# robotic-vision-lab/Dual-Interactive-Implicit-Neural-Network

Hardware: AMD Instinct MI355X
Metric: decoded Mpixels/sec (DIINN implicit decoder, x4 on 256^2 LR) (higher is better)
Workload: dtype f32

## Files before the change

dual-interactive-implicit-neural-network_amd/_native.py:

```python
from __future__ import annotations

import ctypes as C
import os
import threading

PKG_DIR = os.path.dirname(os.path.abspath(__file__))
LIB_PATH = os.environ.get("DIINN_HIP_LIB") or os.path.join(PKG_DIR, "libdiinn_hip.so")

DIINN_OK = 0
ERR_INVALID_ARG, ERR_UNSUPPORTED, ERR_HIP, ERR_TOO_LARGE = 1, 2, 3, 4
SIN_ACCURATE = 0
SIN_HW = 1
SIN_HW_REDUCED = 2
SIN_DEFAULT = SIN_HW_REDUCED
ABI_VERSION = 10
PACKED_MAGIC = 0x44493038
PACKED_MAGIC_WPU = 0x44495750
P_ALGO_DIRECT, P_ALGO_WINOGRAD, P_ALGO_DIRECT_BF16, P_ALGO_DIRECT_BF16X3 = 0, 1, 2, 3
RDN_ALGO_AUTO, RDN_ALGO_DIRECT, RDN_ALGO_WINO, RDN_ALGO_WINO4, RDN_ALGO_X3 = 0, 1, 2, 3, 4
COMPUTE_F32 = 0
COMPUTE_BF16 = 1
COMPUTE_F32_QONLY = 2
COMPUTE_BF16_FULL = 3
COMPUTE_BF16X3 = 4
# ... 56 lines not shown
    "diinn_metasr_decode": (C.c_int, [C.c_void_p, C.c_void_p, C.c_void_p, C.c_void_p, C.c_void_p,
                                      C.c_int, C.c_int, C.c_int, C.c_int, C.c_int]),
    "diinn_metasr_make_axis_tables": (C.c_int, [C.c_int, C.c_int, _i32, _f, _f]),
    "diinn_conv_ksplit": (C.c_int, [C.c_void_p, C.c_void_p, C.c_longlong, C.c_int, C.c_int, C.c_void_p, C.c_void_p,
                                   C.c_void_p, C.c_longlong, C.c_void_p, C.c_longlong, C.c_void_p, C.c_longlong,
                                   C.c_int, C.c_int, C.c_int, C.c_int]),
    "diinn_rdn_packed_floats": (C.c_size_t, []),
    "diinn_rdn_planes_floats": (C.c_size_t, [C.c_int, C.c_int, C.c_int, C.c_int]),
    "diinn_rdn_forward_ex": (C.c_int, [C.c_void_p, C.c_int, C.c_void_p, C.c_void_p, C.c_void_p, C.c_void_p, C.c_void_p, C.c_void_p,
                                       C.c_void_p, C.c_void_p, C.c_void_p, C.c_int, C.c_int, C.c_int]),
    "diinn_conv_wino4_ws_status": (C.c_int, [C.c_void_p, C.c_void_p, C.c_int, _ip]),
    "diinn_sfe1_forward": (C.c_int, [C.c_void_p, C.c_void_p, C.c_int, C.c_void_p, C.c_void_p, C.c_void_p,
                                    C.c_int, C.c_int, C.c_int]),
    "diinn_conv_wino": (C.c_int, [C.c_void_p, C.c_void_p, C.c_longlong, C.c_int, C.c_void_p, C.c_void_p,
                                 C.c_void_p, C.c_longlong, C.c_void_p, C.c_longlong, C.c_int, C.c_int, C.c_int, C.c_int]),
    "diinn_conv3x3_x3": (C.c_int, [C.c_void_p, C.c_void_p, C.c_longlong, C.c_int, C.c_void_p, C.c_void_p,
                                   C.c_void_p, C.c_longlong, C.c_void_p, C.c_longlong, C.c_int, C.c_int, C.c_int, C.c_int]),
    "diinn_rdn_x3_packed_floats": (C.c_size_t, []),
    "diinn_conv_t16": (C.c_int, [C.c_void_p, C.c_void_p, C.c_longlong, C.c_int, C.c_void_p, C.c_void_p,
                                C.c_void_p, C.c_longlong, C.c_void_p, C.c_longlong, C.c_int, C.c_int, C.c_int, C.c_int]),
    "diinn_conv_t16_applies": (C.c_int, [C.c_int, C.c_int, C.c_int]),
    "diinn_conv_t16_plan": (C.c_int, [C.c_int, C.c_int, C.c_int, C.POINTER(C.c_int)]),
    "diinn_conv1x1_t16": (C.c_int, [C.c_void_p, C.c_void_p, C.c_longlong, C.c_int, C.c_void_p, C.c_void_p,
                                   C.c_void_p, C.c_longlong, C.c_void_p, C.c_longlong, C.c_void_p, C.c_longlong,
                                   C.c_int, C.c_int, C.c_int, C.c_int]),
    "diinn_rdn_wino_packed_floats": (C.c_size_t, []),
    "diinn_conv_wino4": (C.c_int, [C.c_void_p, C.c_void_p, C.c_longlong, C.c_int, C.c_void_p, C.c_void_p,
                                  C.c_void_p, C.c_longlong, C.c_void_p, C.c_longlong, C.c_int, C.c_int, C.c_int, C.c_int]),
    "diinn_conv_wino4_ws": (C.c_int, [C.c_void_p, C.c_void_p, C.c_longlong, C.c_int, C.c_void_p, C.c_void_p,
                                     C.c_void_p, C.c_longlong, C.c_void_p, C.c_longlong, C.c_int, C.c_int, C.c_int, C.c_int,
                                     C.c_void_p, C.c_size_t]),
    "diinn_conv_wino4_workspace_floats": (C.c_size_t, []),
    "diinn_conv_wino4_plan": (C.c_int, [C.c_int, C.c_int, C.c_int, C.c_int, C.c_int, C.POINTER(C.c_int)]),
    "diinn_rdn_wino4_packed_floats": (C.c_size_t, []),
    "diinn_rdn_wino4_applies": (C.c_int, [C.c_int, C.c_int, C.c_int]),
    "diinn_liif_decode": (C.c_int, [C.c_void_p, C.c_void_p, C.c_void_p, C.c_void_p, C.c_void_p,
                                    C.c_int, C.c_int, C.c_int, C.c_int, C.c_int]),
    "diinn_liif_make_axis_tables": (C.c_int, [C.c_int, C.c_int, C.c_int, _i32, _f, _f]),
    "diinn_backward_data": (C.c_int, [C.c_void_p, C.c_void_p, C.c_void_p, C.c_void_p, C.c_void_p, C.c_void_p,
                                      C.c_longlong]),
    "diinn_plane_gemm_nt": (C.c_int, [C.c_void_p, C.c_void_p, C.c_int, C.c_int, C.c_void_p, C.c_int, C.c_int,
                                      C.c_void_p, C.c_int, C.c_int, C.c_longlong, C.c_int, C.c_int]),
    "diinn_plane_rowdot": (C.c_int, [C.c_void_p, C.c_void_p, C.c_int, C.c_void_p, C.c_void_p, C.c_int,
                                     C.c_longlong, C.c_int]),
    "diinn_backward_cell_sum": (C.c_int, [C.c_void_p, C.c_void_p, C.c_void_p, C.c_void_p, C.c_void_p,
                                          C.c_int, C.c_int, C.c_int, C.c_int, C.c_int]),
    "diinn_sum_parts": (C.c_int, [C.c_void_p, C.c_void_p, C.c_void_p, C.c_int, C.c_int, C.c_longlong]),
    "diinn_backward_cell_sum_ex": (C.c_int, [C.c_void_p, C.c_void_p, C.c_void_p, C.c_void_p, C.c_void_p, C.c_void_p,
                                             C.c_int, C.c_int, C.c_int, C.c_int, C.c_int]),
    "diinn_unfold_tiled": (C.c_int, [C.c_void_p, C.c_void_p, C.c_void_p, C.c_int, C.c_int, C.c_int, C.c_int]),
    "diinn_training_plane_floats": (C.c_longlong, [C.c_longlong, C.c_int]),
    "diinn_decode_train_fwd": (C.c_int, [C.c_void_p, C.c_void_p, C.c_void_p, C.c_void_p, C.c_void_p,
                                         C.c_int, C.c_int, C.c_int, C.c_int, C.c_int, C.c_int]),
}

_lib = None
_lock = threading.Lock()


class DiinnNativeError(RuntimeError):
    pass


def load() -> C.CDLL:
    global _lib
    if _lib is not None:
# ... 45 lines not shown
```

dual-interactive-implicit-neural-network_amd/csrc/diinn_device.h:

```cpp
#pragma once
#include <hip/hip_runtime.h>
#include <stdint.h>

#include "../../include/diinn_hip.h"
#include "diinn_layout.h"
#include "diinn_knobs.h"

using namespace diinn;

typedef float f32x4 __attribute__((ext_vector_type(4)));
typedef float f32x16 __attribute__((ext_vector_type(16)));
typedef float f32x2 __attribute__((ext_vector_type(2)));
typedef unsigned u32x2 __attribute__((ext_vector_type(2)));
template <int N> struct IC { static constexpr int value = N; };

#define MFMA32(a, b, c) __builtin_amdgcn_mfma_f32_32x32x2f32((a), (b), (c), 0, 0, 0)

template <int MODE>
__device__ __forceinline__ float dsin(float x);

template <>
__device__ __forceinline__ float dsin<DIINN_SIN_ACCURATE>(float x) {
    const float k = __builtin_rintf(x * 0.31830988618379067154f);
    float r = __builtin_fmaf(k, -3.14159274101257324219f, x);
// ... 117 lines not shown
}
struct BlockXYZ { int x, y, z; };
__device__ __forceinline__ BlockXYZ xcd_run_block() {
    const unsigned gx = gridDim.x, gy = gridDim.y;
    const unsigned total = gx * gy * gridDim.z, full = total & ~7u;
    const unsigned lin = blockIdx.x + gx * (blockIdx.y + gy * blockIdx.z);
    const unsigned t = lin < full ? (lin & 7u) * (full >> 3) + (lin >> 3) : lin;
    const unsigned z = t / (gx * gy), r = t - z * gx * gy, y = r / gx;
    return BlockXYZ{__builtin_amdgcn_readfirstlane((int)(r - y * gx)), __builtin_amdgcn_readfirstlane((int)y), __builtin_amdgcn_readfirstlane((int)z)};
}

__device__ __forceinline__ void st_b128(f32x4 v, __amdgpu_buffer_rsrc_t rsrc, unsigned voff, unsigned soff) {
    __builtin_amdgcn_raw_buffer_store_b128(__builtin_bit_cast(u32x4, v), rsrc, (int)voff, (int)soff, 0);
    asm volatile("s_nop 1" ::"v"(v[0]), "v"(v[1]), "v"(v[2]), "v"(v[3]));
}
__device__ __forceinline__ float ld_act(__amdgpu_buffer_rsrc_t rsrc, unsigned voff, unsigned soff) {
    return __builtin_bit_cast(float, __builtin_amdgcn_raw_buffer_load_b32(rsrc, (int)voff, (int)soff, 0));
}
__device__ __forceinline__ __amdgpu_buffer_rsrc_t tile_rsrc(const float* group, long long tile, int rows) {
    return __builtin_amdgcn_make_buffer_rsrc((void*)(group + (size_t)tile * rows * PLANE_TILE), 0,
                                             rows * (int)PLANE_ROW_BYTES, 0x00020000);
}

typedef __bf16 bf16x8 __attribute__((ext_vector_type(8)));
#define MFMA_BF16(a, b, c) __builtin_amdgcn_mfma_f32_32x32x16_bf16((a), (b), (c), 0, 0, 0)

__attribute__((visibility("hidden"))) extern thread_local int g_last_hip_error;
#ifdef DIINN_STAMPS
extern unsigned long long* g_stamps;
#endif

__attribute__((visibility("hidden"))) int device_cus();
__attribute__((visibility("hidden"))) double w4_rounds(long long total, bool have_ws);

static inline int hip_status(hipError_t e) {
    if (e == hipSuccess) return DIINN_OK;
    g_last_hip_error = (int)e;
    return DIINN_ERR_HIP;
}

static inline bool compute_ok(int compute) {
    return compute == DIINN_COMPUTE_F32 || compute == DIINN_COMPUTE_BF16 || compute == DIINN_COMPUTE_F32_QONLY ||
           compute == DIINN_COMPUTE_BF16_FULL || compute == DIINN_COMPUTE_BF16X3;
}

__device__ __forceinline__ int div_m(int x, int d, unsigned m) { return m ? (int)(((unsigned long long)(unsigned)x * m) >> 32) : x / d; }
static inline unsigned magic_m(long long d, long long x_max) { return (d > 1 && d < 65536 && x_max < 65536) ? (unsigned)((1ull << 32) / (unsigned long long)d + 1) : 0u; }
static inline int check_dims(int B, int H, int W) {
    if (B <= 0 || H <= 0 || W <= 0) return DIINN_ERR_INVALID_ARG;
    if ((double)B * H * W * PCH >= 9.0e18 || B > 65535 || H > 65535) return DIINN_ERR_TOO_LARGE;
    return DIINN_OK;
}

static inline int check_window(int row0, int rows, int full, int need0, int need1) {
    if (row0 < 0 || rows <= 0 || row0 > full - rows) return DIINN_ERR_INVALID_ARG;
    if (need0 < row0 || need1 > row0 + rows) return DIINN_ERR_INVALID_ARG;
    return DIINN_OK;
}

static inline int check_npix(long long npix) {
    if (npix <= 0) return DIINN_ERR_INVALID_ARG;
    if (npix > DIINN_TRAIN_MAX_PIXELS) return DIINN_ERR_TOO_LARGE;
    return DIINN_OK;
}

struct RowWin { int row0, rows; };
// ... 26 lines not shown
```

dual-interactive-implicit-neural-network_amd/csrc/diinn_encoder.hip:

```cpp
#include "diinn_device.h"

constexpr int CS_WAVES = 8;
constexpr int CS_TW = 8, CS_TH = 4;
constexpr int CS_HALO = (CS_TH + 2) * (CS_TW + 2);
constexpr int CS_STAGE_FLOATS = 2048;

struct TagFalse { static constexpr bool value = false; };
struct TagTrue { static constexpr bool value = true; };

struct ConvKsplitParams {
    const float* in;
    const float* w;
    const float* bias;
    const float* res;
    float* out0;
    float* out1;
    long long in_bs, out0_bs, out1_bs, res_bs;
    int Cin, B, H, W, relu;
    unsigned m_per_image, m_tiles_x;
#ifdef DIINN_STAMPS
    unsigned long long* stamps;
#endif
};

// ... 575 lines not shown

int diinn_rdn_forward_ex(void* stream, int algo, const float* sfe1_dev, const float* packed_dev, const float* packed_wino_dev,
                         const float* packed_wino4_dev, const float* packed_x3_dev, const float* biases_dev,
                         float* planes, float* w4ws, float* out_dev, int B, int H, int W) {
    switch (algo) {
        case DIINN_RDN_ALGO_AUTO: packed_x3_dev = nullptr; break;
        case DIINN_RDN_ALGO_DIRECT: packed_wino_dev = packed_wino4_dev = packed_x3_dev = nullptr; break;
        case DIINN_RDN_ALGO_WINO:
            if (!packed_wino_dev) return DIINN_ERR_INVALID_ARG;
            packed_wino4_dev = packed_x3_dev = nullptr;
            break;
        case DIINN_RDN_ALGO_WINO4:
            if (!packed_wino4_dev) return DIINN_ERR_INVALID_ARG;
            packed_x3_dev = nullptr;
            break;
        case DIINN_RDN_ALGO_X3:
            if (!packed_wino_dev || !packed_x3_dev) return DIINN_ERR_INVALID_ARG;
            packed_wino4_dev = nullptr;
            break;
        default: return DIINN_ERR_INVALID_ARG;
    }
    if ((((size_t)planes) & 15) || (((size_t)w4ws) & 15)) return DIINN_ERR_INVALID_ARG;
    if (!sfe1_dev || !packed_dev || !biases_dev || !planes || !out_dev) return DIINN_ERR_INVALID_ARG;
    int st = check_dims(B, H, W);
    if (st) return st;
    const long long hw = (long long)H * W;
    const long long wino_min = knob(diinn_knobs().enc_wino_min);
    const bool wino = (packed_wino_dev || packed_wino4_dev) && (long long)B * hw >= wino_min;
    const bool wino4 = packed_wino4_dev && wino && diinn_rdn_wino4_applies(B, H, W);
    if (wino && !wino4 && !packed_wino_dev) return DIINN_ERR_INVALID_ARG;
    const size_t w4ws_floats = w4ws ? diinn_conv_wino4_workspace_floats() : 0;
    if (wino4 && w4ws) {
        st = hip_status(hipMemsetAsync(w4ws, 0, DIINN_WINO4_COUNTER_BYTES, (hipStream_t)stream));
        if (st) return st;
    }
    float* buf[2] = {planes, planes + (size_t)B * 576 * hw};
    float* gff_in = planes + (size_t)2 * B * 576 * hw;
    float* tmp = gff_in + (size_t)B * 1024 * hw;
    const bool x3 = packed_x3_dev && (long long)B * hw >= knob(diinn_knobs().enc_x3_min);
    const bool t16 = !wino && !x3 && diinn_conv_t16_applies(B, H, W) != 0 &&
                     ((((size_t)sfe1_dev) | ((size_t)planes) | ((size_t)packed_dev)) & 15) == 0;
    RdnWeights wt{packed_dev, packed_wino_dev, packed_wino4_dev, packed_x3_dev, biases_dev};
    auto conv = [&](const float* in, long long in_bs, int cin, int taps, const float* res, long long res_bs,
                    float* o0, long long o0_bs, float* o1, long long o1_bs, int relu) {
        const RdnWeights::Slices l = wt.next(cin, taps);
        return (x3 && taps == 9 && !o1)
            ? diinn_conv3x3_x3(stream, in, in_bs, cin, l.wx, l.bias, res, res_bs, o0, o0_bs, relu, B, H, W)
            : (wino4 && taps == 9 && !o1)
            ? diinn_conv_wino4_ws(stream, in, in_bs, cin, l.wu4, l.bias, res, res_bs, o0, o0_bs, relu, B, H, W, w4ws, w4ws_floats)
            : (wino && taps == 9 && !o1)
            ? diinn_conv_wino(stream, in, in_bs, cin, l.wu, l.bias, res, res_bs, o0, o0_bs, relu, B, H, W)
            : (t16 && taps == 9 && !o1)
            ? diinn_conv_t16(stream, in, in_bs, cin, l.w, l.bias, res, res_bs, o0, o0_bs, relu, B, H, W)
            : (t16 && taps == 1 && cin <= 640)
            ? diinn_conv1x1_t16(stream, in, in_bs, cin, l.w, l.bias, res, res_bs, o0, o0_bs, o1, o1_bs, relu, B, H, W)
            : diinn_conv_ksplit(stream, in, in_bs, cin, taps, l.w, l.bias, res, res_bs, o0, o0_bs, o1, o1_bs, relu, B, H, W);
    };
    float* xs = tmp + (size_t)B * 64 * hw;
    const long long xs_bs16 = 144 * hw;
    if (x3) {
        const RdnWeights::Slices l = wt.next(64, 9);
        st = diinn_conv3x3_x3_split(stream, sfe1_dev, 64 * hw, xs, xs_bs16, 0, 64, l.wx, l.bias, buf[0], 576 * hw, 0, B, H, W);
    } else {
        st = conv(sfe1_dev, 64 * hw, 64, 9, nullptr, 0, buf[0], 576 * hw, nullptr, 0, 0);
    }
    if (st) return st;
    for (int d = 0; d < 16; ++d) {
        float* cur = buf[d & 1];
        float* nxt = buf[(d + 1) & 1];
        if (x3) {
            for (int c = 0; c < 8; ++c) {
                const RdnWeights::Slices l = wt.next(64 * (c + 1), 9);
                st = diinn_conv3x3_x3_split(stream, nullptr, 0, xs, xs_bs16, 8 * (c + 1), 64 * (c + 1), l.wx, l.bias,
                                            nullptr, 0, 1, B, H, W);
                if (st) return st;
            }
            const RdnWeights::Slices l = wt.next(576, 1);
            st = diinn_conv1x1_x3_split(stream, xs, xs_bs16, 576, l.wx, l.bias, cur, 576 * hw, nxt, 576 * hw,
                                        gff_in + (size_t)64 * d * hw, 1024 * hw, B, H, W);
            if (st) return st;
            continue;
        }
        for (int c = 0; c < 8; ++c) {
            st = conv(cur, 576 * hw, 64 * (c + 1), 9, nullptr, 0, cur + (size_t)64 * (c + 1) * hw, 576 * hw, nullptr, 0, 1);
            if (st) return st;
        }
        st = conv(cur, 576 * hw, 576, 1, cur, 576 * hw, nxt, 576 * hw, gff_in + (size_t)64 * d * hw, 1024 * hw, 0);
        if (st) return st;
    }
    st = conv(gff_in, 1024 * hw, 1024, 1, nullptr, 0, tmp, 64 * hw, nullptr, 0, 0);
    if (st) return st;
    return conv(tmp, 64 * hw, 64, 9, sfe1_dev, 64 * hw, out_dev, 64 * hw, nullptr, 0, 0);
}

}
```

dual-interactive-implicit-neural-network_amd/csrc/diinn_winograd4.hip:

```cpp
#include "diinn_device.h"

constexpr int W4_TX = 32;
constexpr int W4_THREADS = 1024;
constexpr int W4_VBUF = 36 * 256;
constexpr int W4_RAW0 = 3 * W4_VBUF;
constexpr int W4_RAW_WAVE = 6 * 256 + 64;
constexpr int W4_LDS_FLOATS = W4_RAW0 + 2 * 4 * W4_RAW_WAVE;
static_assert(W4_LDS_FLOATS >= 36 * 1024 && W4_LDS_FLOATS * 4 <= 160 * 1024, "LDS budget");
constexpr int W4_PIECE_BYTES = 1024;
static_assert(3 * W4_VBUF <= W4_LDS_FLOATS, "ring inside the exchange buffer");

#pragma clang diagnostic ignored "-Winline-asm"
#define W4_SB() __builtin_amdgcn_sched_barrier(0)
typedef int i32x4 __attribute__((ext_vector_type(4)));
__device__ __forceinline__ i32x4 w4_rsrc(const void* ptr, unsigned bytes) {
    const unsigned long long a = (unsigned long long)ptr;
    return i32x4{(int)(unsigned)a, (int)((unsigned)(a >> 32) & 0xffffu), (int)bytes, 0x00020000};
}

struct ConvWino4Params {
    const float* in;
    const float* wu;
    const float* bias;
    const float* res;
// ... 43 lines not shown
static_assert(DIINN_WINO4_MAX_SPLIT_WGS <= W4_READY, "one ticket and one ready word per split item");

struct W4Split { int parts, item, slab, first_pair, pair, blk_item; };

__device__ __forceinline__ void w4_st_sc1(f32x4 v, __amdgpu_buffer_rsrc_t rsrc, unsigned voff) {
    __builtin_amdgcn_raw_buffer_store_b128(__builtin_bit_cast(u32x4, v), rsrc, (int)voff, 0, 16);
}
__device__ __forceinline__ f32x4 w4_ld_sc1(__amdgpu_buffer_rsrc_t rsrc, unsigned voff) {
    return __builtin_bit_cast(f32x4, __builtin_amdgcn_raw_buffer_load_b128(rsrc, (int)voff, 0, 16));
}

template <typename T>
__device__ __forceinline__ void w4_bt(const T d0, const T d1, const T d2, const T d3, const T d4, const T d5,
                                      T& r0, T& r1, T& r2, T& r3, T& r4, T& r5) {
    const T a = __builtin_elementwise_fma(T(-4.0f), d2, d4), b = __builtin_elementwise_fma(T(-4.0f), d1, d3);
    const T c = d4 - d2, e = d3 - d1;
    r0 = __builtin_elementwise_fma(T(4.0f), d0, __builtin_elementwise_fma(T(-5.0f), d2, d4));
    r1 = a + b;
    r2 = a - b;
    r3 = __builtin_elementwise_fma(T(2.0f), e, c);
    r4 = __builtin_elementwise_fma(T(-2.0f), e, c);
    r5 = __builtin_elementwise_fma(T(4.0f), d1, __builtin_elementwise_fma(T(-5.0f), d3, d5));
}
template <typename T>
__device__ __forceinline__ void w4_at(const T m0, const T m1, const T m2, const T m3, const T m4, const T m5,
                                      T& y0, T& y1, T& y2, T& y3) {
    const T s = m1 + m2, d = m1 - m2, u = m3 + m4, v = m3 - m4;
    y0 = (m0 + s) + u;
    y1 = __builtin_elementwise_fma(T(2.0f), v, d);
    y2 = __builtin_elementwise_fma(T(4.0f), u, s);
    y3 = __builtin_elementwise_fma(T(8.0f), v, d) + m5;
}

__device__ __forceinline__ void conv_wino4_body(const ConvWino4Params& p, float* __restrict__ lds, int b, int blk, int hh0,
                                                int c0, int m, const W4Split sk) {
    const int tiles_x = (p.W + 3) / 4, tiles_n = tiles_x * ((p.H + 3) / 4);
    auto tile_xy = [&](int tile, int& tx, int& ty) {
        ty = div_m(tile, tiles_x, p.m_tiles_x);
        tx = tile - ty * tiles_x;
        return tile < tiles_n;
    };
    const int lane = threadIdx.x & 63;
    const int wave = __builtin_amdgcn_readfirstlane(threadIdx.x >> 6);
    const size_t plane = (size_t)p.H * p.W;
    const unsigned plane_b = (unsigned)(plane * sizeof(float));
    const int n = p.Cin / 8;
    constexpr unsigned OUTSIDE = 0x80000000u;
    const bool ragged = (p.W & 3) != 0;

    const bool producer = (wave & 3) == 3;
    const int wt_ = wave >> 2, mw = (wave >> 2) * 3 + (wave & 3);
    if (threadIdx.x == 0) W4_STAMP(0, 76, 0);
    if (producer) {
        const int wt = wt_;
        __builtin_amdgcn_s_setprio(3);
        const int th = lane >> 5, tm = lane & 31;
        int ptx, pty;
        const bool pin = tile_xy(blk * W4_TX + tm, ptx, pty);
        (void)pin;
        const bool first = tm == 0, last = tm == W4_TX - 1;
        const bool row_start = ptx == 0, row_end = 4 * ptx + 4 >= p.W;
        const bool ok1 = 4 * ptx + 1 < p.W, ok2 = 4 * ptx + 2 < p.W, ok3 = 4 * ptx + 3 < p.W;
        float* __restrict__ raw = lds + W4_RAW0 + wt * W4_RAW_WAVE;
        const float* __restrict__ in_b = p.in + (size_t)b * p.in_bs;
        unsigned voff[6], voffe;
        {
            const int ek = lane % 6, ew = lane / 6;
            int etx, ety;
// ... 41 lines not shown
                w4_bt<f32x2>(d[0][j], d[1][j], d[2][j], d[3][j], d[4][j], d[5][j], t[0][j], t[1][j], t[2][j], t[3][j], t[4][j], t[5][j]);
            float* __restrict__ dst = vb + (2 * wt + th) * 32 + tm;
#pragma unroll
            for (int i = 0; i < 6; ++i) {
                float v0, v1, v2, v3, v4, v5;
                w4_bt<float>(t[i][0][0], t[i][0][1], t[i][1][0], t[i][1][1], t[i][2][0], t[i][2][1], v0, v1, v2, v3, v4, v5);
                dst[(6 * i + 0) * 256] = v0;
                dst[(6 * i + 1) * 256] = v1;
                dst[(6 * i + 2) * 256] = v2;
                dst[(6 * i + 3) * 256] = v3;
                dst[(6 * i + 4) * 256] = v4;
                dst[(6 * i + 5) * 256] = v5;
            }
        };
        fetch(0, chunk_of(0));
        fetch(1, chunk_of(1));
        asm volatile("s_waitcnt vmcnt(7)\n\ts_barrier" ::: "memory");
        transform(0, lds);
        asm volatile("s_waitcnt lgkmcnt(0)" ::: "memory");
        fetch(0, chunk_of(2));
        asm volatile("s_waitcnt vmcnt(7)\n\ts_barrier" ::: "memory");
        transform(1, lds + W4_VBUF);
        asm volatile("s_waitcnt lgkmcnt(0)" ::: "memory");
        fetch(1, chunk_of(3));
        asm volatile("s_waitcnt vmcnt(7)\n\ts_barrier" ::: "memory");
        int slot2 = 2;
        for (int c = 0; c < m; ++c) {
            if (wt == 0) W4_STAMP(1, c, 0);
            if (c + 2 < m) transform(c & 1, lds + slot2 * W4_VBUF);
            slot2 = slot2 == 2 ? 0 : slot2 + 1;
            asm volatile("s_waitcnt lgkmcnt(0)" ::: "memory");
            fetch(c & 1, chunk_of(c + 4));
            if (wt == 0) W4_STAMP(1, c, 1);
            asm volatile("s_waitcnt vmcnt(7)\n\ts_barrier" ::: "memory");
            if (wt == 0) W4_STAMP(1, c, 2);
        }
        asm volatile("s_waitcnt vmcnt(0)" ::: "memory");
        __builtin_amdgcn_s_setprio(0);
        __builtin_amdgcn_s_barrier();
    } else {
        const __amdgpu_buffer_rsrc_t wrs = __builtin_amdgcn_make_buffer_rsrc(
            (void*)(p.wu + (size_t)(mw * 2 + hh0) * n * (3 * W4_PIECE_BYTES / 4)), 0, n * 3 * W4_PIECE_BYTES, 0x00020000);
        const int lane_off = lane * 16;
        const float* __restrict__ bsrc = lds + 3 * mw * 256 + lane;
        f32x16 acc[3];
        f32x4 A[2][3], Bf[1][3];
#pragma unroll
        for (int q = 0; q < 3; ++q)
#pragma unroll
            for (int r = 0; r < 16; ++r) acc[q][r] = 0.0f;
        __builtin_amdgcn_s_barrier();
        __builtin_amdgcn_s_barrier();
#pragma unroll
        for (int q = 0; q < 3; ++q) {
            A[0][q] = ld_piece(wrs, lane_off, (c0 * 3 + q) * W4_PIECE_BYTES);
            A[1][q] = ld_piece(wrs, lane_off, ((c0 + (m > 1 ? 1 : 0)) * 3 + q) * W4_PIECE_BYTES);
        }
        __builtin_amdgcn_s_barrier();
#pragma unroll
        for (int q = 0; q < 3; ++q) Bf[0][q] = f32x4{bsrc[q * 256], bsrc[q * 256 + 64], bsrc[q * 256 + 128], bsrc[q * 256 + 192]};

        if (mw == 0) W4_STAMP(0, 76, 1);
        if (mw == 0) W4_STAMP_RT(1);
        int slot1 = 1;
        auto iter = [&](auto PAR_, int c) {
            constexpr int PAR = decltype(PAR_)::value;
// ... 84 lines not shown
                }
                __hip_atomic_store(p.sk_cnt + sk.item, 0u, __ATOMIC_RELAXED, __HIP_MEMORY_SCOPE_AGENT);
                __hip_atomic_store(p.sk_cnt + W4_READY + sk.item, 0u, __ATOMIC_RELAXED, __HIP_MEMORY_SCOPE_AGENT);
            }
            __syncthreads();
            const bool poisoned = __builtin_bit_cast(unsigned, *(volatile float*)(lds + W4_FLAG + 1)) != 0u;
            if (threadIdx.x == 0) W4_STAMP(0, 78, 0);
            const int mine = sk.pair - sk.first_pair;
            auto part = [&](int k, f32x4 (&v)[4]) {
                if (k == mine) {
#pragma unroll
                    for (int a = 0; a < 4; ++a) v[a] = f32x4{y[a][0], y[a][1], y[a][2], y[a][3]};
                } else {
                    const int pk = sk.first_pair + k;
                    const int jk = sk.blk_item - (pk * p.sk_u) / (n + p.sk_e);
                    const __amdgpu_buffer_rsrc_t rs = __builtin_amdgcn_make_buffer_rsrc(
                        (void*)(p.sk_slabs + (size_t)(2 * (2 * pk + hh0) + jk) * W4_SLAB_FLOATS), 0, W4_SLAB_FLOATS * 4, 0x00020000);
#pragma unroll
                    for (int a = 0; a < 4; ++a) v[a] = w4_ld_sc1(rs, a * 16384u + toff);
                }
            };
            f32x4 s[4], nxt[4];
            part(0, s);
            for (int k = 1; k < sk.parts; ++k) {
                part(k, nxt);
#pragma unroll
                for (int a = 0; a < 4; ++a) s[a] += nxt[a];
            }
#pragma unroll
            for (int a = 0; a < 4; ++a)
#pragma unroll
                for (int x = 0; x < 4; ++x) y[a][x] = poisoned ? __builtin_nanf("") : s[a][x];
            if (threadIdx.x == 0) W4_STAMP(0, 78, 1);
        }
        const int ox = 4 * tx, oy0 = 4 * ty;
        const bool vec = !ragged && (p.out_bs & 3) == 0 && (((size_t)p.out) & 15) == 0 &&
                         (!p.res || ((p.res_bs & 3) == 0 && (((size_t)p.res) & 15) == 0));
        const int co = 32 * hh0 + 8 * (r >> 2) + 4 * h + (r & 3);
        const float bias = p.bias[co];
        float* __restrict__ op = p.out + (size_t)b * p.out_bs + (size_t)co * plane;
        const float* __restrict__ rp = p.res ? p.res + (size_t)b * p.res_bs + (size_t)co * plane : nullptr;
#pragma unroll
        for (int a = 0; a < 4; ++a) {
            const int oy = oy0 + a;
            if (!tin || oy >= p.H || ox >= p.W) continue;
            f32x4 v = {y[a][0] + bias, y[a][1] + bias, y[a][2] + bias, y[a][3] + bias};
            if (p.relu) v = f32x4{relu0(v[0]), relu0(v[1]), relu0(v[2]), relu0(v[3])};
            const size_t o = (size_t)oy * p.W + ox;
            if (vec) {
                if (rp) v += *reinterpret_cast<const f32x4*>(rp + o);
                *reinterpret_cast<f32x4*>(op + o) = v;
            } else {
#pragma unroll
                for (int x = 0; x < 4; ++x)
                    if (ox + x < p.W) op[o + x] = rp ? v[x] + rp[o + x] : v[x];
            }
        }
    }
    if (threadIdx.x == 0) W4_STAMP(0, 76, 3);
}

__global__ __launch_bounds__(W4_THREADS) void conv_wino4_kernel(const ConvWino4Params p) {
    __shared__ __attribute__((aligned(16))) float lds[W4_LDS_FLOATS];
    const int nblk = (((p.W + 3) / 4) * ((p.H + 3) / 4) + W4_TX - 1) / W4_TX;
    const int n = p.Cin / 8;
    if ((int)blockIdx.x < p.sk_wgs) {
        const int g = (int)(blockIdx.x & 7) * (p.sk_wgs >> 3) + (int)(blockIdx.x >> 3);
        const int pair = g >> 1, hh0 = g & 1;
        const int ne = n + p.sk_e;
        const int vtotal = (p.sk_items >> 1) * ne;
        int v0 = pair * p.sk_u;
        const int v1 = v0 + p.sk_u < vtotal ? v0 + p.sk_u : vtotal;
        for (int j = 0; v0 < v1;) {
            const int it = v0 / ne;
            const int rs = it * ne + p.sk_e, be = (it + 1) * ne;
            const int a = v0 > rs ? v0 : rs, e = v1 < be ? v1 : be;
            if (a < e) {
                const int first = rs / p.sk_u, last = (be - 1) / p.sk_u;
                const int t = (p.sk_first >> 1) + it;
                const int b = __builtin_amdgcn_readfirstlane(div_m(t, nblk, p.m_nblk));
                conv_wino4_body(p, lds, b, t - b * nblk, hh0, a - rs, e - a, W4Split{last - first + 1, 2 * it + hh0, 2 * g + j, first, pair, it});
                __syncthreads();
                ++j;
            }
            v0 = be;
        }
        return;
    }
    const int total = p.sk_first;
    const int bid = (int)blockIdx.x - p.sk_wgs;
    const int wg_per_xcd = ((int)gridDim.x - p.sk_wgs) >> 3;
    const int per_xcd = (total + 7) >> 3;
    const int xcd = bid & 7, idx = bid >> 3;
    for (int k = idx; k < per_xcd; k += wg_per_xcd) {
        int t = xcd * per_xcd + k;
        if (t >= total) break;
        const int hh0 = t & 1;
        t >>= 1;
        const int b = __builtin_amdgcn_readfirstlane(div_m(t, nblk, p.m_nblk));
        conv_wino4_body(p, lds, b, t - b * nblk, hh0, 0, n, W4Split{1, 0, 0, 0, 0, 0});
        __syncthreads();
    }
}

#ifdef W4_STAMPS
unsigned long long* g_w4_stamps = nullptr;
#endif

struct W4Plan { int first, items, u, wgs, e; };
static int w4_cus() {
    int ncu = device_cus();
    if (ncu > DIINN_WINO4_MAX_SPLIT_WGS) ncu = DIINN_WINO4_MAX_SPLIT_WGS;
    return ncu & ~1;
}
constexpr int W4_SPLIT_E = 4;
static inline double w4_whole_us(int n) { return 10.0 + 1.46 * n; }
static inline double w4_split_us(int u, int e) { return 17.5 - 1.75 * e + 1.75 * u; }
static W4Plan w4_plan(long long total, int n, int ncu, bool have_ws) {
    W4Plan pl{(int)total, 0, 0, 0, 0};
    const long long mode = knob(diinn_knobs().enc_wino4_split);
    if (!have_ws || mode == 0 || ncu < 8) return pl;
    const int R = (int)(total % ncu);
    if (R == 0) return pl;
    int e = W4_SPLIT_E, ne = n + e;
    int u = (int)(((long long)(R / 2) * ne + ncu / 2 - 1) / (ncu / 2));
    if (u <= e) {
        e = 0; ne = n;
        u = (int)(((long long)(R / 2) * ne + ncu / 2 - 1) / (ncu / 2));
    }
    if (u >= ne) return pl;
    if (mode == 1 && w4_split_us(u, e) > w4_whole_us(n) - 1.0) return pl;
    const int wgs = 2 * (int)(((long long)(R / 2) * ne + u - 1) / u);
    pl.first = (int)(total - R);
    pl.items = R;
    pl.u = u;
    pl.e = e;
    pl.wgs = (wgs + 15) / 16 * 16;
    return pl;
}

__attribute__((visibility("hidden"))) double w4_rounds(long long total, bool have_ws) {
    const int ncu = w4_cus();
    if (ncu < 2) return (double)total;
    const long long whole = total / ncu, R = total % ncu;
    if (R == 0) return (double)whole;
    const W4Plan pl = w4_plan(total, 36, ncu, have_ws);
    const double last = pl.items ? 0.27 + 0.86 * (double)R / ncu : 1.0;
    return (double)whole + (last < 1.0 ? last : 1.0);
}

extern "C" {

size_t diinn_conv_wino4_workspace_floats(void) {
    return (size_t)1024 + (size_t)2 * (DIINN_WINO4_MAX_SPLIT_WGS + 8) * W4_SLAB_FLOATS;
}

int diinn_conv_wino4_ws(void* stream, const float* in_dev, long long in_batch_stride, int Cin,
                        const float* packed_u_dev, const float* bias_dev, const float* res_dev, long long res_batch_stride,
                        float* out_dev, long long out_batch_stride, int relu, int B, int H, int W,
                        float* ws_dev, size_t ws_floats) {
    if (!in_dev || !packed_u_dev || !bias_dev || !out_dev) return DIINN_ERR_INVALID_ARG;
    int st = check_dims(B, H, W);
    if (st) return st;
    if (Cin <= 0 || Cin % 8) return DIINN_ERR_UNSUPPORTED;
    if ((((size_t)in_dev) & 3) || (((size_t)packed_u_dev) & 15) || (((size_t)bias_dev) & 3) || (((size_t)ws_dev) & 15))
        return DIINN_ERR_INVALID_ARG;
    if (ws_dev && ws_floats < diinn_conv_wino4_workspace_floats()) return DIINN_ERR_INVALID_ARG;
    const long long blocks = (((long long)((W + 3) / 4) * ((H + 3) / 4) + W4_TX - 1) / W4_TX) * B;
    if (2 * blocks > 2147483000LL) return DIINN_ERR_TOO_LARGE;
    if ((long long)H * W * 4 * 64 > 0x7FFFFFFFLL) return DIINN_ERR_TOO_LARGE;
    if ((long long)Cin / 8 * 3 * W4_PIECE_BYTES > 0x7FFFFFFFLL) return DIINN_ERR_TOO_LARGE;
    ConvWino4Params p;
    p.in = in_dev; p.wu = packed_u_dev; p.bias = bias_dev; p.res = res_dev; p.out = out_dev;
    p.in_bs = in_batch_stride; p.out_bs = out_batch_stride; p.res_bs = res_batch_stride;
    p.Cin = Cin; p.B = B; p.H = H; p.W = W; p.relu = relu ? 1 : 0;
    {
        const long long tiles_x = (W + 3) / 4, nblk = (tiles_x * ((H + 3) / 4) + W4_TX - 1) / W4_TX;
        p.m_tiles_x = magic_m(tiles_x, nblk * W4_TX);
        p.m_nblk = magic_m(nblk, blocks);
    }
    const W4Plan pl = w4_plan(2 * blocks, Cin / 8, w4_cus(), ws_dev != nullptr);
    p.sk_fault = knob(diinn_knobs().enc_wino4_fault) == 1 ? 1 : 0;
    p.sk_spin_max = p.sk_fault ? (1u << 10) : (1u << 24);
    p.sk_first = pl.first; p.sk_items = pl.items; p.sk_u = pl.u; p.sk_e = pl.e; p.sk_wgs = pl.wgs;
    p.sk_cnt = (unsigned*)ws_dev;
    p.sk_slabs = ws_dev ? ws_dev + 1024 : nullptr;
// ... 5 lines not shown
    return hip_status(hipGetLastError());
}

int diinn_conv_wino4_ws_status(void* stream, float* ws_dev, int clear, int* status) {
    if (!ws_dev || !status) return DIINN_ERR_INVALID_ARG;
    unsigned word = 0;
    int st = hip_status(hipMemcpyAsync(&word, (const unsigned*)ws_dev + W4_STATUS, sizeof(word), hipMemcpyDeviceToHost, (hipStream_t)stream));
    if (st) return st;
    if (clear) {
        st = hip_status(hipMemsetAsync(ws_dev, 0, 4096, (hipStream_t)stream));
        if (st) return st;
    }
    st = hip_status(hipStreamSynchronize((hipStream_t)stream));
    if (st) return st;
    *status = word != 0u ? 1 : 0;
    return DIINN_OK;
}

int diinn_conv_wino4(void* stream, const float* in_dev, long long in_batch_stride, int Cin,
                     const float* packed_u_dev, const float* bias_dev, const float* res_dev, long long res_batch_stride,
                     float* out_dev, long long out_batch_stride, int relu, int B, int H, int W) {
    return diinn_conv_wino4_ws(stream, in_dev, in_batch_stride, Cin, packed_u_dev, bias_dev, res_dev, res_batch_stride,
                               out_dev, out_batch_stride, relu, B, H, W, nullptr, 0);
}

int diinn_conv_wino4_plan(int Cin, int B, int H, int W, int with_workspace, int info[4]) {
    if (!info || Cin <= 0 || Cin % 8 || check_dims(B, H, W)) return DIINN_ERR_INVALID_ARG;
    const long long blocks = (((long long)((W + 3) / 4) * ((H + 3) / 4) + W4_TX - 1) / W4_TX) * B;
    const W4Plan pl = w4_plan(2 * blocks, Cin / 8, w4_cus(), with_workspace != 0);
    info[0] = (int)(2 * blocks); info[1] = pl.first; info[2] = pl.wgs; info[3] = pl.u;
    return DIINN_OK;
}

}
```

dual-interactive-implicit-neural-network_amd/modules.py:

```python
from __future__ import annotations

from types import SimpleNamespace
from typing import Any, Dict, Optional

import torch
import torch.nn as nn
import torch.nn.functional as F

from .decoder import ImplicitDecoder
from .metrics import calc_psnr, psnr, resize_fn, ssim


class RDB_Conv(nn.Module):

    def __init__(self, inChannels: int, growRate: int, kSize: int = 3):
        super().__init__()
        self.conv = nn.Sequential(nn.Conv2d(inChannels, growRate, kSize, padding=(kSize - 1) // 2), nn.ReLU())

    def forward(self, x):
        return torch.cat((x, self.conv(x)), 1)


class RDB(nn.Module):

# ... 157 lines not shown
        if ws is None:
            while len(cls._w4_areas) >= cls._W4_AREAS_MAX:
                cls._w4_areas.pop(next(iter(cls._w4_areas)))
            ws = torch.empty(floats, dtype=torch.float32, device=device)
            ws[:1024].zero_()
            cls._w4_areas[key] = ws
        return ws

    @classmethod
    def handoff_status(cls, clear: bool = True) -> int:
        import ctypes as C
        from . import _native
        lib = _native.load()
        worst = 0
        for (dev, stream), ws in list(cls._w4_areas.items()):
            st = C.c_int(0)
            with torch.cuda.device(ws.device):
                _native.check(lib.diinn_conv_wino4_ws_status(C.c_void_p(stream), C.c_void_p(ws.data_ptr()), int(clear), C.byref(st)),
                              "diinn_conv_wino4_ws_status")
            worst = max(worst, st.value)
        return worst

    def _forward_hip_trunk(self, shallow):
        import ctypes as C
        from . import _native
        lib = _native.load()
        b, _, h, w = shallow.shape
        shallow = shallow.contiguous()
        dev = shallow.device
        packed, biases = self._hip_packed(dev)
        x3 = self.hip_winograd and self.hip_split_bf16
        w4 = self.hip_winograd and self.hip_winograd4 and not x3 and bool(lib.diinn_rdn_wino4_applies(b, h, w))
        needs_wino = self.hip_winograd and not w4 and (x3 or b * h * w >= _native.debug_get("DIINN_ENC_WINO_MIN"))
        algo = (_native.RDN_ALGO_X3 if x3 else _native.RDN_ALGO_WINO4 if w4 else _native.RDN_ALGO_WINO if needs_wino
                else _native.RDN_ALGO_DIRECT)
        ptr = lambda t: C.c_void_p(t.data_ptr()) if t is not None else None
        packed_wino = self._hip_packed_wino(dev) if needs_wino else None
        packed_w4 = self._hip_packed_wino4(dev) if w4 else None
        packed_x3 = self._hip_packed_x3(dev) if x3 else None
        planes = torch.empty(lib.diinn_rdn_planes_floats(algo, b, h, w), dtype=torch.float32, device=dev)
        area = self._w4_area(dev) if w4 else None
        out = torch.empty_like(shallow)
        with torch.cuda.device(dev):
            stream = C.c_void_p(torch.cuda.current_stream().cuda_stream)
            _native.check(lib.diinn_rdn_forward_ex(stream, algo, ptr(shallow), ptr(packed), ptr(packed_wino), ptr(packed_w4),
                                                   ptr(packed_x3), ptr(biases), ptr(planes), ptr(area), ptr(out), b, h, w),
                          "diinn_rdn_forward_ex")
        return out

    def _sfe1_hip(self, x):
        import ctypes as C
        from . import _native
        lib = _native.load()
        x = x.contiguous()
        b, c, h, w = x.shape
        wt, bias = self.SFENet1.weight.detach().contiguous(), self.SFENet1.bias.detach().contiguous()
        out = torch.empty((b, 64, h, w), dtype=torch.float32, device=x.device)
        with torch.cuda.device(x.device):
            stream = C.c_void_p(torch.cuda.current_stream().cuda_stream)
            _native.check(lib.diinn_sfe1_forward(stream, C.c_void_p(x.data_ptr()), c, C.c_void_p(wt.data_ptr()),
                                                 C.c_void_p(bias.data_ptr()), C.c_void_p(out.data_ptr()), b, h, w),
                          "diinn_sfe1_forward")
        return out

    def forward(self, x):
        if (self._hip_ok and self.hip_trunk_max_pixels is not None and x.is_cuda and not torch.is_grad_enabled()
                and x.dtype == torch.float32 and x.shape[0] * x.shape[-2] * x.shape[-1] <= self.hip_trunk_max_pixels):
# ... 304 lines not shown
```

include/diinn_hip.h:

```cpp
#ifndef DIINN_HIP_H
#define DIINN_HIP_H

#include <stddef.h>
#include <stdint.h>

#ifdef __cplusplus
extern "C" {
#endif

#define DIINN_ABI_VERSION 10

#define DIINN_OK                 0
#define DIINN_ERR_INVALID_ARG    1
#define DIINN_ERR_UNSUPPORTED    2
#define DIINN_ERR_HIP            3
#define DIINN_ERR_TOO_LARGE      4

#define DIINN_IN_CHANNELS 64
#define DIINN_HIDDEN      256
#define DIINN_LAYERS      4
#define DIINN_OUT         3
#define DIINN_P_CHANNELS  (DIINN_LAYERS * DIINN_HIDDEN)

#define DIINN_SIN_ACCURATE 0
// ... 110 lines not shown
#define DIINN_RDN_ALGO_WINO   2
#define DIINN_RDN_ALGO_WINO4  3
#define DIINN_RDN_ALGO_X3     4
size_t diinn_rdn_planes_floats(int algo, int B, int H, int W);
int    diinn_rdn_forward_ex(void* stream, int algo, const float* sfe1_dev, const float* packed_dev, const float* packed_wino_dev,
                            const float* packed_wino4_dev, const float* packed_x3_dev, const float* biases_dev,
                            float* planes_dev, float* w4ws_dev, float* out_dev, int B, int H, int W);
int    diinn_conv_ksplit(void* stream, const float* in_dev, long long in_batch_stride, int Cin, int taps,
                        const float* packed_w_dev, const float* bias_dev,
                        const float* res_dev, long long res_batch_stride,
                        float* out0_dev, long long out0_batch_stride, float* out1_dev, long long out1_batch_stride,
                        int relu, int B, int H, int W);
size_t diinn_rdn_packed_floats(void);

int    diinn_sfe1_forward(void* stream, const float* x_dev, int Cin, const float* w_dev, const float* bias_dev,
                          float* out_dev, int B, int H, int W);
int    diinn_conv_wino(void* stream, const float* in_dev, long long in_batch_stride, int Cin,
                      const float* packed_u_dev, const float* bias_dev,
                      const float* res_dev, long long res_batch_stride,
                      float* out_dev, long long out_batch_stride, int relu, int B, int H, int W);
size_t diinn_rdn_wino_packed_floats(void);

int    diinn_conv_wino4(void* stream, const float* in_dev, long long in_batch_stride, int Cin,
                        const float* packed_u_dev, const float* bias_dev,
                        const float* res_dev, long long res_batch_stride,
                        float* out_dev, long long out_batch_stride, int relu, int B, int H, int W);
size_t diinn_conv_wino4_workspace_floats(void);
int    diinn_conv_wino4_ws(void* stream, const float* in_dev, long long in_batch_stride, int Cin,
                           const float* packed_u_dev, const float* bias_dev,
                           const float* res_dev, long long res_batch_stride,
                           float* out_dev, long long out_batch_stride, int relu, int B, int H, int W,
                           float* ws_dev, size_t ws_floats);
int    diinn_conv_wino4_plan(int Cin, int B, int H, int W, int with_workspace, int info[4]);
int    diinn_conv_wino4_ws_status(void* stream, float* ws_dev, int clear, int* status);
#define DIINN_WINO4_MAX_SPLIT_WGS 256
#define DIINN_WINO4_COUNTER_BYTES 2048
size_t diinn_rdn_wino4_packed_floats(void);
int    diinn_rdn_wino4_applies(int B, int H, int W);

int    diinn_conv3x3_x3(void* stream, const float* in_dev, long long in_batch_stride, int Cin,
                        const float* packed_x3_dev, const float* bias_dev,
                        const float* res_dev, long long res_batch_stride,
                        float* out_dev, long long out_batch_stride, int relu, int B, int H, int W);
size_t diinn_rdn_x3_packed_floats(void);

int    diinn_conv_t16(void* stream, const float* in_dev, long long in_batch_stride, int Cin,
                      const float* packed_w_dev, const float* bias_dev,
                      const float* res_dev, long long res_batch_stride,
                      float* out_dev, long long out_batch_stride, int relu, int B, int H, int W);
int    diinn_conv_t16_applies(int B, int H, int W);
int    diinn_conv_t16_plan(int B, int H, int W, int info[4]);
int    diinn_conv1x1_t16(void* stream, const float* in_dev, long long in_batch_stride, int Cin,
                         const float* packed_w_dev, const float* bias_dev,
                         const float* res_dev, long long res_batch_stride,
                         float* out0_dev, long long out0_batch_stride, float* out1_dev, long long out1_batch_stride,
                         int relu, int B, int H, int W);

int diinn_decode_launch_info(int B, int Hu, int Wu, int y0, int y1,
                             int* grid_x, int* grid_y, int* grid_z, int* block);
#define DIINN_DECODE_KERNEL_THROUGHPUT 1
#define DIINN_DECODE_KERNEL_LATENCY16  3
#define DIINN_DECODE_KERNEL_OTHER      0
int diinn_decode_kernel_info(int B, int Hu, int Wu, int y0, int y1, int x0, int x1, int compute, int info[4]);
#define DIINN_P_ALGO_DIRECT      0
#define DIINN_P_ALGO_WINOGRAD    1
#define DIINN_P_ALGO_DIRECT_BF16 2
// ... 12 lines not shown
```

Measured before the change: 172.6.

## Fuse dense-block Winograd-4 convs into one persistent kernel with tile-level dataflow sync

```diff
diff --git a/dual-interactive-implicit-neural-network_amd/_native.py b/dual-interactive-implicit-neural-network_amd/_native.py
--- a/dual-interactive-implicit-neural-network_amd/_native.py
+++ b/dual-interactive-implicit-neural-network_amd/_native.py
@@ -112,6 +112,7 @@
                                      C.c_void_p, C.c_size_t]),
     "diinn_conv_wino4_workspace_floats": (C.c_size_t, []),
     "diinn_conv_wino4_plan": (C.c_int, [C.c_int, C.c_int, C.c_int, C.c_int, C.c_int, C.POINTER(C.c_int)]),
+    "diinn_conv_wino4_rdb_plan": (C.c_int, [C.c_int, C.c_int, C.c_int, C.c_int, C.c_int, C.POINTER(C.c_int)]),
     "diinn_rdn_wino4_packed_floats": (C.c_size_t, []),
     "diinn_rdn_wino4_applies": (C.c_int, [C.c_int, C.c_int, C.c_int]),
     "diinn_liif_decode": (C.c_int, [C.c_void_p, C.c_void_p, C.c_void_p, C.c_void_p, C.c_void_p,
diff --git a/dual-interactive-implicit-neural-network_amd/csrc/diinn_device.h b/dual-interactive-implicit-neural-network_amd/csrc/diinn_device.h
--- a/dual-interactive-implicit-neural-network_amd/csrc/diinn_device.h
+++ b/dual-interactive-implicit-neural-network_amd/csrc/diinn_device.h
@@ -173,6 +173,9 @@
 
 __attribute__((visibility("hidden"))) int device_cus();
 __attribute__((visibility("hidden"))) double w4_rounds(long long total, bool have_ws);
+__attribute__((visibility("hidden"))) int w4_rdb_applies(int B, int H, int W, const float* ws_dev, size_t* ready_off, size_t* ready_bytes);
+__attribute__((visibility("hidden"))) int w4_rdb_launch(void* stream, float* buf, long long bs, const float* const wu[8],
+                                                        const float* const bias[8], int B, int H, int W, float* ws_dev, int d);
 
 static inline int hip_status(hipError_t e) {
     if (e == hipSuccess) return DIINN_OK;
diff --git a/dual-interactive-implicit-neural-network_amd/csrc/diinn_encoder.hip b/dual-interactive-implicit-neural-network_amd/csrc/diinn_encoder.hip
--- a/dual-interactive-implicit-neural-network_amd/csrc/diinn_encoder.hip
+++ b/dual-interactive-implicit-neural-network_amd/csrc/diinn_encoder.hip
@@ -631,6 +631,13 @@
     const size_t w4ws_floats = w4ws ? diinn_conv_wino4_workspace_floats() : 0;
     if (wino4 && w4ws) {
         st = hip_status(hipMemsetAsync(w4ws, 0, DIINN_WINO4_COUNTER_BYTES, (hipStream_t)stream));
+        if (st) return st;
+    }
+    size_t rdb_off = 0, rdb_bytes = 0;
+    const bool rdb = algo == DIINN_RDN_ALGO_AUTO && wino4 && w4ws && (hw & 3) == 0 &&
+                     w4_rdb_applies(B, H, W, w4ws, &rdb_off, &rdb_bytes) != 0;
+    if (rdb) {
+        st = hip_status(hipMemsetAsync(w4ws + rdb_off, 0, rdb_bytes, (hipStream_t)stream));
         if (st) return st;
     }
     float* buf[2] = {planes, planes + (size_t)B * 576 * hw};
@@ -680,6 +687,15 @@
             if (st) return st;
             continue;
         }
+        if (rdb) {
+            const float *wu4[8], *bias[8];
+            for (int c = 0; c < 8; ++c) {
+                const RdnWeights::Slices l = wt.next(64 * (c + 1), 9);
+                wu4[c] = l.wu4; bias[c] = l.bias;
+            }
+            st = w4_rdb_launch(stream, cur, 576 * hw, wu4, bias, B, H, W, w4ws, d);
+            if (st) return st;
+        } else
         for (int c = 0; c < 8; ++c) {
             st = conv(cur, 576 * hw, 64 * (c + 1), 9, nullptr, 0, cur + (size_t)64 * (c + 1) * hw, 576 * hw, nullptr, 0, 1);
             if (st) return st;
diff --git a/dual-interactive-implicit-neural-network_amd/csrc/diinn_winograd4.hip b/dual-interactive-implicit-neural-network_amd/csrc/diinn_winograd4.hip
--- a/dual-interactive-implicit-neural-network_amd/csrc/diinn_winograd4.hip
+++ b/dual-interactive-implicit-neural-network_amd/csrc/diinn_winograd4.hip
@@ -99,8 +99,30 @@
     y3 = __builtin_elementwise_fma(T(8.0f), v, d) + m5;
 }
 
+__host__ __device__ __forceinline__ void w4_rdb_reach(int blk, int tiles_x, int tiles_n, int& lo, int& hi) {
+    lo = blk * W4_TX - tiles_x - 1;
+    hi = blk * W4_TX + W4_TX + tiles_x;
+    lo = lo < 0 ? 0 : lo / W4_TX;
+    hi = (hi < tiles_n ? hi : tiles_n - 1) / W4_TX;
+}
+__host__ __device__ __forceinline__ int w4_whole_item(int bid, int k, int grid, int total) {
+    const int per_xcd = (total + 7) >> 3, i = (bid >> 3) + k * (grid >> 3);
+    const int t = (bid & 7) * per_xcd + i;
+    return i < per_xcd && t < total ? t : -1;
+}
+struct W4Rdb {
+    const unsigned* wait;
+    unsigned* post;
+    unsigned* status;
+    unsigned target;
+    unsigned spin_max;
+    int wait_chunk;
+};
+constexpr int W4_POISON = W4_LDS_FLOATS;
+
+template <bool RDB>
 __device__ __forceinline__ void conv_wino4_body(const ConvWino4Params& p, float* __restrict__ lds, int b, int blk, int hh0,
-                                                int c0, int m, const W4Split sk) {
+                                                int c0, int m, const W4Split sk, const W4Rdb rdb) {
     const int tiles_x = (p.W + 3) / 4, tiles_n = tiles_x * ((p.H + 3) / 4);
     auto tile_xy = [&](int tile, int& tx, int& ty) {
         ty = div_m(tile, tiles_x, p.m_tiles_x);
@@ -208,6 +230,27 @@
             asm volatile("s_waitcnt lgkmcnt(0)" ::: "memory");
             fetch(c & 1, chunk_of(c + 4));
             if (wt == 0) W4_STAMP(1, c, 1);
+            if constexpr (RDB) {
+                if (rdb.wait && c + 5 == rdb.wait_chunk && wt == 0) {
+                    const int nblk = (tiles_n + W4_TX - 1) / W4_TX;
+                    int lo, hi;
+                    w4_rdb_reach(blk, tiles_x, tiles_n, lo, hi);
+                    const unsigned* word = rdb.wait + (size_t)b * nblk + lo + (lane <= hi - lo ? lane : 0);
+                    unsigned spins = 0;
+                    while (__builtin_amdgcn_ballot_w64(__hip_atomic_load(word, __ATOMIC_RELAXED, __HIP_MEMORY_SCOPE_AGENT) < rdb.target) != 0) {
+                        __builtin_amdgcn_s_sleep(4);
+                        if (++spins > rdb.spin_max) {
+                            if (lane == 0) {
+                                __hip_atomic_store(rdb.status + W4_STATUS, 1u, __ATOMIC_RELAXED, __HIP_MEMORY_SCOPE_AGENT);
+                                lds[W4_POISON] = __builtin_bit_cast(float, 1u);
+                            }
+                            break;
+                        }
+                    }
+                    __builtin_amdgcn_fence(__ATOMIC_ACQUIRE, "agent");
+                    asm volatile("s_waitcnt vmcnt(0)" ::: "memory");
+                }
+            }
             asm volatile("s_waitcnt vmcnt(7)\n\ts_barrier" ::: "memory");
             if (wt == 0) W4_STAMP(1, c, 2);
         }
@@ -358,6 +401,31 @@
 #pragma unroll
                 for (int x = 0; x < 4; ++x) y[a][x] = poisoned ? __builtin_nanf("") : s[a][x];
             if (threadIdx.x == 0) W4_STAMP(0, 78, 1);
+        }
+        if constexpr (RDB) {
+            const bool poisoned = __builtin_bit_cast(unsigned, *(volatile float*)(lds + W4_POISON)) != 0u;
+            const int co_w = 32 * hh0 + 8 * (r >> 2) + (r & 3);
+            const float bias = p.bias[co_w + 4 * h];
+            const __amdgpu_buffer_rsrc_t ors = __builtin_amdgcn_make_buffer_rsrc(
+                (void*)(p.out + (size_t)b * p.out_bs + (size_t)co_w * plane), 0, (int)(5u * plane_b), 0x00020000);
+            const unsigned obase = (unsigned)(4 * h) * plane_b + (unsigned)((4 * ty) * p.W + 4 * tx) * 4u;
+#pragma unroll
+            for (int a = 0; a < 4; ++a) {
+                if (!tin || 4 * ty + a >= p.H) continue;
+                f32x4 v = {y[a][0] + bias, y[a][1] + bias, y[a][2] + bias, y[a][3] + bias};
+                if (p.relu) v = f32x4{relu0(v[0]), relu0(v[1]), relu0(v[2]), relu0(v[3])};
+                if (poisoned) v = f32x4{__builtin_nanf(""), __builtin_nanf(""), __builtin_nanf(""), __builtin_nanf("")};
+                w4_st_sc1(v, ors, obase + (unsigned)(a * p.W) * 4u);
+            }
+            if (rdb.post) {
+                asm volatile("s_waitcnt vmcnt(0)" ::: "memory");
+                __syncthreads();
+                if (threadIdx.x == 0) {
+                    const int nblk = (tiles_n + W4_TX - 1) / W4_TX;
+                    __hip_atomic_fetch_add(rdb.post + (size_t)b * nblk + blk, 1u, __ATOMIC_RELAXED, __HIP_MEMORY_SCOPE_AGENT);
+                }
+            }
+            return;
         }
         const int ox = 4 * tx, oy0 = 4 * ty;
         const bool vec = !ragged && (p.out_bs & 3) == 0 && (((size_t)p.out) & 15) == 0 &&
@@ -405,7 +473,7 @@
                 const int first = rs / p.sk_u, last = (be - 1) / p.sk_u;
                 const int t = (p.sk_first >> 1) + it;
                 const int b = __builtin_amdgcn_readfirstlane(div_m(t, nblk, p.m_nblk));
-                conv_wino4_body(p, lds, b, t - b * nblk, hh0, a - rs, e - a, W4Split{last - first + 1, 2 * it + hh0, 2 * g + j, first, pair, it});
+                conv_wino4_body<false>(p, lds, b, t - b * nblk, hh0, a - rs, e - a, W4Split{last - first + 1, 2 * it + hh0, 2 * g + j, first, pair, it}, W4Rdb{});
                 __syncthreads();
                 ++j;
             }
@@ -424,8 +492,42 @@
         const int hh0 = t & 1;
         t >>= 1;
         const int b = __builtin_amdgcn_readfirstlane(div_m(t, nblk, p.m_nblk));
-        conv_wino4_body(p, lds, b, t - b * nblk, hh0, 0, n, W4Split{1, 0, 0, 0, 0, 0});
+        conv_wino4_body<false>(p, lds, b, t - b * nblk, hh0, 0, n, W4Split{1, 0, 0, 0, 0, 0}, W4Rdb{});
         __syncthreads();
+    }
+}
+
+struct W4RdbLayer { const float* wu; const float* bias; float* out; int Cin, pad; };
+constexpr int W4_RDB_LAYERS = 8;
+struct ConvWino4RdbParams {
+    ConvWino4Params p;
+    W4RdbLayer layer[W4_RDB_LAYERS];
+    unsigned* ready;
+    unsigned* status;
+    unsigned target, spin_max;
+    int layers, nb;
+};
+__global__ __launch_bounds__(W4_THREADS) void conv_wino4_rdb_kernel(const ConvWino4RdbParams P) {
+    __shared__ __attribute__((aligned(16))) float lds[W4_LDS_FLOATS + 4];
+    const int nblk = (((P.p.W + 3) / 4) * ((P.p.H + 3) / 4) + W4_TX - 1) / W4_TX;
+    if (threadIdx.x == 0)
+        lds[W4_POISON] = __builtin_bit_cast(float, __hip_atomic_load(P.status + W4_STATUS, __ATOMIC_RELAXED, __HIP_MEMORY_SCOPE_AGENT));
+    __syncthreads();
+    for (int l = 0; l < P.layers; ++l) {
+        ConvWino4Params p = P.p;
+        p.wu = P.layer[l].wu; p.bias = P.layer[l].bias; p.out = P.layer[l].out; p.Cin = P.layer[l].Cin;
+        const int n = p.Cin / 8;
+        const W4Rdb rdb{l ? P.ready + (size_t)(l - 1) * P.nb : nullptr, l + 1 < P.layers ? P.ready + (size_t)l * P.nb : nullptr,
+                        P.status, P.target, P.spin_max, n - 8};
+        for (int k = 0;; ++k) {
+            int t = w4_whole_item((int)blockIdx.x, k, (int)gridDim.x, p.sk_first);
+            if (t < 0) break;
+            const int hh0 = t & 1;
+            t >>= 1;
+            const int b = __builtin_amdgcn_readfirstlane(div_m(t, nblk, p.m_nblk));
+            conv_wino4_body<true>(p, lds, b, t - b * nblk, hh0, 0, n, W4Split{1, 0, 0, 0, 0, 0}, rdb);
+            __syncthreads();
+        }
     }
 }
 
@@ -475,9 +577,81 @@
     return (double)whole + (last < 1.0 ? last : 1.0);
 }
 
+struct W4RdbPlan { int grid, items, nblk, nb; };
+constexpr size_t W4_RDB_READY0 = (size_t)1024 + (size_t)2 * DIINN_WINO4_MAX_SPLIT_WGS * W4_SLAB_FLOATS;
+constexpr size_t W4_RDB_READY_WORDS = (size_t)2 * 8 * W4_SLAB_FLOATS;
+static W4RdbPlan w4_rdb_plan(int B, int H, int W, int ncu) {
+    W4RdbPlan pl{0, 0, 0, 0};
+    if (B <= 0 || H <= 0 || W <= 0 || (W & 3)) return pl;
+    const long long tiles_x = (W + 3) / 4, tiles_n = tiles_x * ((H + 3) / 4), nblk = (tiles_n + W4_TX - 1) / W4_TX;
+    const long long nb = nblk * B;
+    if (2 * nb > 2147483000LL || (size_t)(W4_RDB_LAYERS - 1) * (size_t)nb > W4_RDB_READY_WORDS) return pl;
+    if ((long long)H * W * 4 * 64 > 0x7FFFFFFFLL) return pl;
+    if ((2 * tiles_x + 2 + 2 * W4_TX - 1) / W4_TX + 1 > 64) return pl;
+    for (int c = 1; c <= W4_RDB_LAYERS; ++c)
+        if (w4_plan(2 * nb, 8 * c, ncu, true).items) return pl;
+    const long long grid = (2 * nb + 7) / 8 * 8 < (ncu & ~7) ? (2 * nb + 7) / 8 * 8 : (ncu & ~7);
+    if (grid < 8) return pl;
+    pl.grid = (int)grid; pl.items = (int)(2 * nb); pl.nblk = (int)nblk; pl.nb = (int)nb;
+    return pl;
+}
+static int w4_rdb_resident() {
+    static std::atomic<int> cache[64];
+    int dev = 0;
+    if (hipGetDevice(&dev) != hipSuccess || dev < 0 || dev >= 64) return 0;
+    int n = cache[dev].load(std::memory_order_relaxed);
+    if (n == 0) {
+        int cus = 0, per_cu = 0;
+        if (hipDeviceGetAttribute(&cus, hipDeviceAttributeMultiprocessorCount, dev) != hipSuccess || cus <= 0) return 0;
+        if (hipOccupancyMaxActiveBlocksPerMultiprocessor(&per_cu, conv_wino4_rdb_kernel, W4_THREADS, 0) != hipSuccess || per_cu <= 0) return 0;
+        n = cus;
+        cache[dev].store(n, std::memory_order_relaxed);
+    }
+    return n;
+}
+__attribute__((visibility("hidden"))) int w4_rdb_applies(int B, int H, int W, const float* ws_dev, size_t* ready_off, size_t* ready_bytes) {
+    if (!ws_dev) return 0;
+    const W4RdbPlan pl = w4_rdb_plan(B, H, W, w4_cus());
+    if (!pl.grid || pl.grid > w4_rdb_resident()) return 0;
+    *ready_off = W4_RDB_READY0;
+    *ready_bytes = (size_t)(W4_RDB_LAYERS - 1) * pl.nb * sizeof(unsigned);
+    return 1;
+}
+__attribute__((visibility("hidden"))) int w4_rdb_launch(void* stream, float* buf, long long bs, const float* const wu[8],
+                                                        const float* const bias[8], int B, int H, int W, float* ws_dev, int d) {
+    const W4RdbPlan pl = w4_rdb_plan(B, H, W, w4_cus());
+    if (!pl.grid || !ws_dev || !buf || (((size_t)buf) & 15) || (bs & 3) || d < 0 || pl.grid > w4_rdb_resident()) return DIINN_ERR_INVALID_ARG;
+    ConvWino4RdbParams P;
+    ConvWino4Params& p = P.p;
+    p.in = buf; p.wu = nullptr; p.bias = nullptr; p.res = nullptr; p.out = nullptr;
+    p.in_bs = bs; p.out_bs = bs; p.res_bs = 0;
+    p.Cin = 0; p.B = B; p.H = H; p.W = W; p.relu = 1;
+    p.m_tiles_x = magic_m((W + 3) / 4, (long long)pl.nblk * W4_TX);
+    p.m_nblk = magic_m(pl.nblk, pl.nb);
+    p.sk_slabs = nullptr; p.sk_cnt = nullptr;
+    p.sk_first = pl.items; p.sk_items = 0; p.sk_u = 0; p.sk_e = 0; p.sk_wgs = 0; p.sk_spin_max = 0; p.sk_fault = 0;
+#ifdef W4_STAMPS
+    p.stamps = g_w4_stamps;
+#endif
+    const size_t plane = (size_t)H * W;
+    for (int c = 0; c < W4_RDB_LAYERS; ++c) {
+        if (!wu[c] || !bias[c] || (((size_t)wu[c]) & 15)) return DIINN_ERR_INVALID_ARG;
+        P.layer[c] = W4RdbLayer{wu[c], bias[c], buf + (size_t)64 * (c + 1) * plane, 64 * (c + 1), 0};
+    }
+    P.ready = (unsigned*)(ws_dev + W4_RDB_READY0);
+    P.status = (unsigned*)ws_dev;
+    P.target = 2u * (unsigned)(d + 1);
+    P.spin_max = 1u << 24;
+    P.layers = W4_RDB_LAYERS;
+    P.nb = pl.nb;
+    hipLaunchKernelGGL(conv_wino4_rdb_kernel, dim3((unsigned)pl.grid), dim3(W4_THREADS), 0, (hipStream_t)stream, P);
+    return hip_status(hipGetLastError());
+}
+
 extern "C" {
 
 size_t diinn_conv_wino4_workspace_floats(void) {
+    static_assert(W4_RDB_READY0 + W4_RDB_READY_WORDS == (size_t)1024 + (size_t)2 * (DIINN_WINO4_MAX_SPLIT_WGS + 8) * W4_SLAB_FLOATS, "the READY words of the dense-block kernel");
     return (size_t)1024 + (size_t)2 * (DIINN_WINO4_MAX_SPLIT_WGS + 8) * W4_SLAB_FLOATS;
 }
 
@@ -549,4 +723,18 @@
     return DIINN_OK;
 }
 
-}
+int diinn_conv_wino4_rdb_plan(int B, int H, int W, int wg, int k, int info[6]) {
+    if (!info || check_dims(B, H, W)) return DIINN_ERR_INVALID_ARG;
+    const W4RdbPlan pl = w4_rdb_plan(B, H, W, w4_cus());
+    info[0] = pl.grid; info[1] = pl.items; info[2] = pl.nblk; info[3] = -1; info[4] = info[5] = 0;
+    if (pl.grid && wg >= 0 && wg < pl.grid && k >= 0) {
+        info[3] = w4_whole_item(wg, k, pl.grid, pl.items);
+        if (info[3] >= 0) {
+            const int tiles_x = (W + 3) / 4, tiles_n = tiles_x * ((H + 3) / 4);
+            w4_rdb_reach((info[3] >> 1) % pl.nblk, tiles_x, tiles_n, info[4], info[5]);
+        }
+    }
+    return DIINN_OK;
+}
+
+}
diff --git a/dual-interactive-implicit-neural-network_amd/modules.py b/dual-interactive-implicit-neural-network_amd/modules.py
--- a/dual-interactive-implicit-neural-network_amd/modules.py
+++ b/dual-interactive-implicit-neural-network_amd/modules.py
@@ -213,7 +213,7 @@
         x3 = self.hip_winograd and self.hip_split_bf16
         w4 = self.hip_winograd and self.hip_winograd4 and not x3 and bool(lib.diinn_rdn_wino4_applies(b, h, w))
         needs_wino = self.hip_winograd and not w4 and (x3 or b * h * w >= _native.debug_get("DIINN_ENC_WINO_MIN"))
-        algo = (_native.RDN_ALGO_X3 if x3 else _native.RDN_ALGO_WINO4 if w4 else _native.RDN_ALGO_WINO if needs_wino
+        algo = (_native.RDN_ALGO_X3 if x3 else _native.RDN_ALGO_AUTO if w4 else _native.RDN_ALGO_WINO if needs_wino
                 else _native.RDN_ALGO_DIRECT)
         ptr = lambda t: C.c_void_p(t.data_ptr()) if t is not None else None
         packed_wino = self._hip_packed_wino(dev) if needs_wino else None
diff --git a/include/diinn_hip.h b/include/diinn_hip.h
--- a/include/diinn_hip.h
+++ b/include/diinn_hip.h
@@ -166,6 +166,7 @@
                            float* out_dev, long long out_batch_stride, int relu, int B, int H, int W,
                            float* ws_dev, size_t ws_floats);
 int    diinn_conv_wino4_plan(int Cin, int B, int H, int W, int with_workspace, int info[4]);
+int    diinn_conv_wino4_rdb_plan(int B, int H, int W, int wg, int k, int info[6]);
 int    diinn_conv_wino4_ws_status(void* stream, float* ws_dev, int clear, int* status);
 #define DIINN_WINO4_MAX_SPLIT_WGS 256
 #define DIINN_WINO4_COUNTER_BYTES 2048
```

Measured after the change: 172.4 (median of 2 runs). No clear change (-0.1%).
